# 86885974647565434342125458569795756674/torch.distributed.pipeline.sync.Pipe

Measured on AMD Instinct MI355X. Metric: tokens/sec for 12-layer Transformer at PP=N (pipeline-parallel training), higher is better.
Workload: dtype bf16

## Files before the change

### mipipe/csrc/kernels/attention.hip

```cpp
#include <type_traits>

#include "common.h"
#include "kernels.h"

namespace mipipe {

namespace {

typedef __attribute__((ext_vector_type(4))) short s16x4;
typedef __attribute__((ext_vector_type(8))) short s16x8;
typedef __attribute__((address_space(3))) s16x4 lds_s16x4;

constexpr int kRows = 64;
constexpr int kThreads = 256;
constexpr float kLog2e = 1.4426950408889634f;

template <int D>
struct Img {
  static constexpr int kRowBytes = 2 * D;
  static constexpr int kChunks = D / 8;
  static constexpr int kBytes = kRows * kRowBytes;
  __device__ static __forceinline__ int f(int r) {
    if constexpr (kChunks >= 16) return (((r ^ (r >> 2)) & 1) << 1) | ((r & 2) << 1) | (r & 8);
    else if constexpr (kChunks == 8) return ((((r >> 1) ^ (r >> 2)) & 1) << 1) | ((r >> 1) & 4);
    else return (((r & 3) << 2) | ((r >> 2) & 3)) & (kChunks - 1);
  }
  __device__ static __forceinline__ int off(int r, int c16) { return r * kRowBytes + ((c16 ^ f(r)) << 4); }
};

template <int D>
__device__ __forceinline__ void stage_tile(const bf16_t* __restrict__ base, int64_t ld, char* img, int tid) {
  constexpr int kPer = kRows * Img<D>::kChunks / kThreads;
#pragma unroll
  for (int u = 0; u < kPer; ++u) {
    const int id = tid + u * kThreads;
    const int r = id / Img<D>::kChunks, c = id % Img<D>::kChunks;
    const uint4 v = *reinterpret_cast<const uint4*>(base + (int64_t)r * ld + c * 8);
    *reinterpret_cast<uint4*>(img + Img<D>::off(r, c)) = v;
  }
}

struct TileRegs {
  uint4 r0, r1, r2, r3;
};
template <int D>
__device__ __forceinline__ uint4 load_piece(const bf16_t* __restrict__ base, int64_t ld, int tid, int u) {
  const int id = tid + u * kThreads;
  const int r = id / Img<D>::kChunks, c = id % Img<D>::kChunks;
  return *reinterpret_cast<const uint4*>(base + (int64_t)r * ld + c * 8);
}
template <int D>
__device__ __forceinline__ void store_piece(char* img, int tid, int u, const uint4& v) {
  const int id = tid + u * kThreads;
// ... 904 lines not shown
        float dp = pacc[j][r];
        float pdrop = pr;
        if (a.p > 0.f) {
          const uint32_t w = r == 0 ? kw0 : (r == 1 ? kw1 : (r == 2 ? kw2 : kw3));
          const bool keep = w >= a.threshold;
          pdrop = keep ? pr * pscale : 0.f;
          dp = keep ? dp * pscale : 0.f;
        }
        pd[j][r] = pdrop;
        ds[j][r] = pr * (dp - dl);
        if constexpr (SOFTCAP) ds[j][r] *= dcap;
      }
    }
    scratch_write(scr, pd, lane);
    __builtin_amdgcn_s_waitcnt(0xC07F);
    bf16x8 f0 = scratch_frag(scr, 0, lane);
    bf16x8 f1 = scratch_frag(scr, 1, lane);
#pragma unroll
    for (int t2 = 0; t2 < ND; ++t2) {
      dv[t2] = __builtin_amdgcn_mfma_f32_16x16x32_bf16(f0, frag_cols<D>(dimg, 16 * t2, 0, lane), dv[t2], 0, 0, 0);
      dv[t2] = __builtin_amdgcn_mfma_f32_16x16x32_bf16(f1, frag_cols<D>(dimg, 16 * t2, 1, lane), dv[t2], 0, 0, 0);
    }
    __builtin_amdgcn_s_waitcnt(0xC07F);
    scratch_write(scr, ds, lane);
    __builtin_amdgcn_s_waitcnt(0xC07F);
    f0 = scratch_frag(scr, 0, lane);
    f1 = scratch_frag(scr, 1, lane);
#pragma unroll
    for (int t2 = 0; t2 < ND; ++t2) {
      dk[t2] = __builtin_amdgcn_mfma_f32_16x16x32_bf16(f0, frag_cols<D>(qimg, 16 * t2, 0, lane), dk[t2], 0, 0, 0);
      dk[t2] = __builtin_amdgcn_mfma_f32_16x16x32_bf16(f1, frag_cols<D>(qimg, 16 * t2, 1, lane), dk[t2], 0, 0, 0);
    }
  }
  const DkvDst dst = dkv_dst<0>(blockIdx.y);
  bf16_t* dK = dst.dk;
  bf16_t* dV = dst.dv;
#pragma unroll
  for (int t2 = 0; t2 < ND; ++t2)
#pragma unroll
    for (int r = 0; r < 4; ++r) {
      const int64_t o = (int64_t)(key0 + r) * dst.ld + 16 * t2 + (lane & 15);
      dK[o] = f2bf(dk[t2][r] * a.scale);
      dV[o] = f2bf(dv[t2][r]);
    }
}

namespace shortseq {

constexpr int S = 128;
constexpr int kThreads = 512;
constexpr int kChunk = 64;
constexpr int kChunkImg = S * kChunk * 2;
constexpr int kSqImg = S * S * 2;
constexpr int kStageBytes = 3 * kChunkImg;
constexpr int kPOff = 4 * kChunkImg;
constexpr int kDsOff = kPOff + kSqImg;
constexpr int kSmem = kDsOff + kSqImg;
constexpr int kFwdPOff = 2 * kChunkImg;
constexpr int kFwdSmem = kFwdPOff + kSqImg;

__device__ __forceinline__ int coff(int r, int c16) { return Img<64>::off(r, c16); }
__device__ __forceinline__ int soff(int r, int c16) { return Img<128>::off(r, c16); }

__device__ __forceinline__ void load_chunk(const bf16_t* __restrict__ base, int64_t ld, int d0, int tid, uint4& v0,
                                           uint4& v1) {
  const int r = tid >> 3, c = tid & 7;
  v0 = *reinterpret_cast<const uint4*>(base + (int64_t)r * ld + d0 + 8 * c);
  v1 = *reinterpret_cast<const uint4*>(base + (int64_t)(r + 64) * ld + d0 + 8 * c);
}
__device__ __forceinline__ void store_chunk(char* img, int tid, const uint4& v0, const uint4& v1) {
  const int r = tid >> 3, c = tid & 7;
  *reinterpret_cast<uint4*>(img + coff(r, c)) = v0;
  *reinterpret_cast<uint4*>(img + coff(r + 64, c)) = v1;
}

__device__ __forceinline__ bf16x8 crow(const char* img, int rb, int s, int lane) {
  return *reinterpret_cast<const bf16x8*>(img + coff(rb + (lane & 15), 4 * s + (lane >> 4)));
}
__device__ __forceinline__ bf16x8 ccol(const char* img, int db, int s, int lane) {
  const int g = lane >> 4, q = (lane & 15) >> 2, p = lane & 3;
  const int r0 = 32 * s + 8 * g + q;
  const int c8 = (db >> 2) + p;
  const int o0 = coff(r0, c8 >> 1) + 8 * (c8 & 1);
  const int o1 = coff(r0 + 4, c8 >> 1) + 8 * (c8 & 1);
  const s16x4 lo = __builtin_amdgcn_ds_read_tr16_b64_v4i16((lds_s16x4*)(img + o0));
  const s16x4 hi = __builtin_amdgcn_ds_read_tr16_b64_v4i16((lds_s16x4*)(img + o1));
  return __builtin_bit_cast(bf16x8, __builtin_shufflevector(lo, hi, 0, 1, 2, 3, 4, 5, 6, 7));
}
__device__ __forceinline__ bf16x8 srow(const char* img, int rb, int s, int lane) {
  return *reinterpret_cast<const bf16x8*>(img + soff(rb + (lane & 15), 4 * s + (lane >> 4)));
}
__device__ __forceinline__ bf16x8 scol(const char* img, int ib, int s, int lane) {
  const int g = lane >> 4, q = (lane & 15) >> 2, p = lane & 3;
  const int r0 = 32 * s + 8 * g + q;
  const int c8 = (ib >> 2) + p;
  const int o0 = soff(r0, c8 >> 1) + 8 * (c8 & 1);
  const int o1 = soff(r0 + 4, c8 >> 1) + 8 * (c8 & 1);
  const s16x4 lo = __builtin_amdgcn_ds_read_tr16_b64_v4i16((lds_s16x4*)(img + o0));
  const s16x4 hi = __builtin_amdgcn_ds_read_tr16_b64_v4i16((lds_s16x4*)(img + o1));
  return __builtin_bit_cast(bf16x8, __builtin_shufflevector(lo, hi, 0, 1, 2, 3, 4, 5, 6, 7));
}

template <int D, bool CAUSAL>
__global__ void __launch_bounds__(kThreads, 1) attn_bwd_s128_kernel(AttnArgs a) {
  extern __shared__ __attribute__((aligned(16))) char smem[];
  const int tid = threadIdx.x, lane = tid & 63, wave = __builtin_amdgcn_readfirstlane(tid >> 6);
  const int bh = blockIdx.x;
  const int b = bh / a.H, h = bh % a.H;
  const int64_t boff = (int64_t)b * a.sb_qkv + (int64_t)h * a.sh_qkv;
  const int64_t koff = (int64_t)b * a.sb_qkv + (int64_t)kv_head(a, h) * a.sh_qkv;
  const bf16_t* Q = reinterpret_cast<const bf16_t*>(a.q) + boff;
  const bf16_t* K = reinterpret_cast<const bf16_t*>(a.k) + koff;
  const bf16_t* V = reinterpret_cast<const bf16_t*>(a.v) + koff;
  const bf16_t* dO = reinterpret_cast<const bf16_t*>(a.dout) + (int64_t)b * a.sb_o + (int64_t)h * a.sh_o;
  constexpr int NC = D / kChunk;

  f32x4 sacc[8], pacc[8];
#pragma unroll
  for (int j = 0; j < 8; ++j) sacc[j] = pacc[j] = f32x4{0.f, 0.f, 0.f, 0.f};
  const int myrow = wave * 16 + (lane & 15);
  const bf16_t* qrow = Q + (int64_t)myrow * a.ld_qkv;
  const bf16_t* drow = dO + (int64_t)myrow * a.ld_o;

  uint4 k0, k1, v0, v1;
  load_chunk(K, a.ld_qkv, 0, tid, k0, k1);
  load_chunk(V, a.ld_qkv, 0, tid, v0, v1);
  store_chunk(smem, tid, k0, k1);
  store_chunk(smem + kChunkImg, tid, v0, v1);
  __syncthreads();
#pragma unroll 1
  for (int c = 0; c < NC; ++c) {
    const char* kimg = smem + (c & 1) * 2 * kChunkImg;
    const char* vimg = kimg + kChunkImg;
    if (c + 1 < NC) {
      load_chunk(K, a.ld_qkv, (c + 1) * kChunk, tid, k0, k1);
      load_chunk(V, a.ld_qkv, (c + 1) * kChunk, tid, v0, v1);
    }
    bf16x8 qf[2], df[2];
#pragma unroll
    for (int s2 = 0; s2 < 2; ++s2) {
      qf[s2] = frag_global(qrow + c * kChunk, s2, lane);
      df[s2] = frag_global(drow + c * kChunk, s2, lane);
    }
#pragma unroll
    for (int s2 = 0; s2 < 2; ++s2)
#pragma unroll
      for (int j = 0; j < 8; ++j) {
        sacc[j] = __builtin_amdgcn_mfma_f32_16x16x32_bf16(qf[s2], crow(kimg, 16 * j, s2, lane), sacc[j], 0, 0, 0);
        pacc[j] = __builtin_amdgcn_mfma_f32_16x16x32_bf16(df[s2], crow(vimg, 16 * j, s2, lane), pacc[j], 0, 0, 0);
      }
    if (c + 1 < NC) {
      char* nimg = smem + ((c + 1) & 1) * 2 * kChunkImg;
      store_chunk(nimg, tid, k0, k1);
      store_chunk(nimg + kChunkImg, tid, v0, v1);
    }
    __syncthreads();
  }

  const int qrow0 = wave * 16 + 4 * (lane >> 4);
  const float sl2 = a.scale * kLog2e;
  const float pscale = a.p > 0.f ? 1.f / (1.f - a.p) : 1.f;
  float lse2[4];
#pragma unroll
  for (int r = 0; r < 4; ++r) lse2[r] = a.lse[(int64_t)bh * S + qrow0 + r] * kLog2e;
  float dsum[4] = {0.f, 0.f, 0.f, 0.f};
#pragma unroll
  for (int j = 0; j < 8; ++j) {
    const int key = 16 * j + (lane & 15);
    uint32_t w[4] = {0xFFFFFFFFu, 0xFFFFFFFFu, 0xFFFFFFFFu, 0xFFFFFFFFu};
    if (a.p > 0.f) {
      const uint4 mw = attn_mask_words(a, bh, qrow0 >> 2, key);
      w[0] = mw.x; w[1] = mw.y; w[2] = mw.z; w[3] = mw.w;
    }
#pragma unroll
    for (int r = 0; r < 4; ++r) {
      float pr = __builtin_amdgcn_exp2f(sacc[j][r] * sl2 - lse2[r]);
      if (CAUSAL && key > qrow0 + r) pr = 0.f;
      float dp = pacc[j][r];
      float pd = pr;
      if (a.p > 0.f) {
        const bool keep = w[r] >= a.threshold;
        dp = keep ? dp * pscale : 0.f;
        pd = keep ? pr * pscale : 0.f;
      }
      sacc[j][r] = pr;
      pacc[j][r] = dp;
      dsum[r] += pr * dp;
      *reinterpret_cast<bf16_t*>(smem + kPOff + soff(qrow0 + r, key >> 3) + 2 * (key & 7)) = f2bf(pd);
    }
  }
  float delta[4];
#pragma unroll
  for (int r = 0; r < 4; ++r) delta[r] = row_reduce_sum16(dsum[r]);
#pragma unroll
  for (int j = 0; j < 8; ++j) {
    const int key = 16 * j + (lane & 15);
#pragma unroll
    for (int r = 0; r < 4; ++r) {
      const float ds = sacc[j][r] * (pacc[j][r] - delta[r]);
      *reinterpret_cast<bf16_t*>(smem + kDsOff + soff(qrow0 + r, key >> 3) + 2 * (key & 7)) = f2bf(ds);
    }
  }

  const char* pimg = smem + kPOff;
  const char* dsimg = smem + kDsOff;
  char* kimg = smem;
  char* qimg = smem + kChunkImg;
  char* dimg = smem + 2 * kChunkImg;
  const int r0 = wave * 16;
  uint4 a0, a1, b0, b1, e0, e1;
  load_chunk(K, a.ld_qkv, 0, tid, a0, a1);
  load_chunk(Q, a.ld_qkv, 0, tid, b0, b1);
  load_chunk(dO, a.ld_o, 0, tid, e0, e1);
#pragma unroll 1
  for (int c = 0; c < NC; ++c) {
    const int d0 = c * kChunk;
    __syncthreads();
    store_chunk(kimg, tid, a0, a1);
    store_chunk(qimg, tid, b0, b1);
    store_chunk(dimg, tid, e0, e1);
    __syncthreads();
    if (c + 1 < NC) {
      load_chunk(K, a.ld_qkv, d0 + kChunk, tid, a0, a1);
      load_chunk(Q, a.ld_qkv, d0 + kChunk, tid, b0, b1);
      load_chunk(dO, a.ld_o, d0 + kChunk, tid, e0, e1);
    }
    f32x4 dq[4], dk[4], dv[4];
#pragma unroll
    for (int t = 0; t < 4; ++t) dq[t] = dk[t] = dv[t] = f32x4{0.f, 0.f, 0.f, 0.f};
#pragma unroll
    for (int ks = 0; ks < 4; ++ks) {
      const bf16x8 a_dq = srow(dsimg, r0, ks, lane);
      const bf16x8 a_dk = scol(dsimg, r0, ks, lane);
      const bf16x8 a_dv = scol(pimg, r0, ks, lane);
#pragma unroll
      for (int t = 0; t < 4; ++t) {
        dq[t] = __builtin_amdgcn_mfma_f32_16x16x32_bf16(a_dq, ccol(kimg, 16 * t, ks, lane), dq[t], 0, 0, 0);
        dk[t] = __builtin_amdgcn_mfma_f32_16x16x32_bf16(a_dk, ccol(qimg, 16 * t, ks, lane), dk[t], 0, 0, 0);
        dv[t] = __builtin_amdgcn_mfma_f32_16x16x32_bf16(a_dv, ccol(dimg, 16 * t, ks, lane), dv[t], 0, 0, 0);
      }
    }
    const int orow = r0 + 4 * (lane >> 4);
    __syncthreads();
#pragma unroll
    for (int t = 0; t < 4; ++t) {
      const int col = 16 * t + (lane & 15);
#pragma unroll
      for (int r = 0; r < 4; ++r) {
        const int at = coff(orow + r, col >> 3) + 2 * (col & 7);
        *reinterpret_cast<bf16_t*>(kimg + at) = f2bf(dq[t][r] * a.scale);
        *reinterpret_cast<bf16_t*>(qimg + at) = f2bf(dk[t][r] * a.scale);
        *reinterpret_cast<bf16_t*>(dimg + at) = f2bf(dv[t][r]);
      }
    }
    __syncthreads();
    {
      const int r = tid >> 3, cc = tid & 7;
      const DkvDst dst = dkv_dst<0>(blockIdx.x);
      bf16_t* dK = dst.dk;
      bf16_t* dV = dst.dv;
      bf16_t* dQ = dq_dst<0>(blockIdx.x);
#pragma unroll
      for (int h2 = 0; h2 < 2; ++h2) {
        const int row = r + 64 * h2;
        const int off = coff(row, cc);
        const int64_t g = (int64_t)row * a.ld_qkv + d0 + 8 * cc;
        const int64_t gk = (int64_t)row * dst.ld + d0 + 8 * cc;
        *reinterpret_cast<uint4*>(dQ + g) = *reinterpret_cast<const uint4*>(kimg + off);
        *reinterpret_cast<uint4*>(dK + gk) = *reinterpret_cast<const uint4*>(qimg + off);
        *reinterpret_cast<uint4*>(dV + gk) = *reinterpret_cast<const uint4*>(dimg + off);
      }
    }
  }
}

template <int D, bool CAUSAL>
__global__ void __launch_bounds__(kThreads, 2) attn_fwd_s128_kernel(AttnArgs a) {
  extern __shared__ __attribute__((aligned(16))) char smem[];
  const int tid = threadIdx.x, lane = tid & 63, wave = __builtin_amdgcn_readfirstlane(tid >> 6);
  const int bh = blockIdx.x;
  const int b = bh / a.H, h = bh % a.H;
  const int64_t boff = (int64_t)b * a.sb_qkv + (int64_t)h * a.sh_qkv;
  const int64_t koff = (int64_t)b * a.sb_qkv + (int64_t)kv_head(a, h) * a.sh_qkv;
  const bf16_t* Q = reinterpret_cast<const bf16_t*>(a.q) + boff;
  const bf16_t* K = reinterpret_cast<const bf16_t*>(a.k) + koff;
  const bf16_t* V = reinterpret_cast<const bf16_t*>(a.v) + koff;
  constexpr int NC = D / kChunk;

  f32x4 sacc[8];
#pragma unroll
  for (int j = 0; j < 8; ++j) sacc[j] = f32x4{0.f, 0.f, 0.f, 0.f};
  const bf16_t* qrow = Q + (int64_t)(wave * 16 + (lane & 15)) * a.ld_qkv;

  uint4 k0, k1;
  load_chunk(K, a.ld_qkv, 0, tid, k0, k1);
  store_chunk(smem, tid, k0, k1);
  __syncthreads();
#pragma unroll 1
  for (int c = 0; c < NC; ++c) {
    const char* kimg = smem + (c & 1) * kChunkImg;
    if (c + 1 < NC) load_chunk(K, a.ld_qkv, (c + 1) * kChunk, tid, k0, k1);
    bf16x8 qf[2];
#pragma unroll
    for (int s2 = 0; s2 < 2; ++s2) qf[s2] = frag_global(qrow + c * kChunk, s2, lane);
#pragma unroll
    for (int s2 = 0; s2 < 2; ++s2)
#pragma unroll
      for (int j = 0; j < 8; ++j)
        sacc[j] = __builtin_amdgcn_mfma_f32_16x16x32_bf16(qf[s2], crow(kimg, 16 * j, s2, lane), sacc[j], 0, 0, 0);
    if (c + 1 < NC) store_chunk(smem + ((c + 1) & 1) * kChunkImg, tid, k0, k1);
    __syncthreads();
  }

  const int qrow0 = wave * 16 + 4 * (lane >> 4);
  const float sl2 = a.scale * kLog2e;
  const float pscale = a.p > 0.f ? 1.f / (1.f - a.p) : 1.f;
  float mx[4] = {-INFINITY, -INFINITY, -INFINITY, -INFINITY};
#pragma unroll
  for (int j = 0; j < 8; ++j) {
    const int key = 16 * j + (lane & 15);
#pragma unroll
    for (int r = 0; r < 4; ++r) {
      float x = sacc[j][r] * sl2;
      if (CAUSAL && key > qrow0 + r) x = -INFINITY;
      sacc[j][r] = x;
      mx[r] = fmaxf(mx[r], x);
    }
  }
#pragma unroll
  for (int r = 0; r < 4; ++r) mx[r] = row_reduce_max16(mx[r]);
  float sum[4] = {0.f, 0.f, 0.f, 0.f};
#pragma unroll
  for (int j = 0; j < 8; ++j)
#pragma unroll
    for (int r = 0; r < 4; ++r) {
      const float e = __builtin_amdgcn_exp2f(sacc[j][r] - mx[r]);
      sacc[j][r] = e;
      sum[r] += e;
    }
  float inv[4];
#pragma unroll
  for (int r = 0; r < 4; ++r) {
    sum[r] = row_reduce_sum16(sum[r]);
    inv[r] = 1.f / sum[r];
  }
  char* pimg = smem + kFwdPOff;
#pragma unroll
  for (int j = 0; j < 8; ++j) {
    const int key = 16 * j + (lane & 15);
    uint32_t w[4] = {0xFFFFFFFFu, 0xFFFFFFFFu, 0xFFFFFFFFu, 0xFFFFFFFFu};
    if (a.p > 0.f) {
      const uint4 mw = attn_mask_words(a, bh, qrow0 >> 2, key);
      w[0] = mw.x; w[1] = mw.y; w[2] = mw.z; w[3] = mw.w;
    }
#pragma unroll
    for (int r = 0; r < 4; ++r) {
      float pv = sacc[j][r] * inv[r];
      if (a.p > 0.f) pv = w[r] >= a.threshold ? pv * pscale : 0.f;
      *reinterpret_cast<bf16_t*>(pimg + soff(qrow0 + r, key >> 3) + 2 * (key & 7)) = f2bf(pv);
    }
  }
  if ((lane & 15) == 0) {
#pragma unroll
    for (int r = 0; r < 4; ++r) a.lse[(int64_t)bh * S + qrow0 + r] = (mx[r] + log2f(sum[r])) / kLog2e;
  }

  bf16_t* O = reinterpret_cast<bf16_t*>(a.o) + (int64_t)b * a.sb_o + (int64_t)h * a.sh_o;
  uint4 v0, v1;
  load_chunk(V, a.ld_qkv, 0, tid, v0, v1);
  store_chunk(smem, tid, v0, v1);
  __syncthreads();
  const int r0 = wave * 16;
#pragma unroll 1
  for (int c = 0; c < NC; ++c) {
    const char* vimg = smem + (c & 1) * kChunkImg;
    if (c + 1 < NC) load_chunk(V, a.ld_qkv, (c + 1) * kChunk, tid, v0, v1);
    f32x4 o[4];
#pragma unroll
    for (int t = 0; t < 4; ++t) o[t] = f32x4{0.f, 0.f, 0.f, 0.f};
#pragma unroll
    for (int ks = 0; ks < 4; ++ks) {
      const bf16x8 ap = srow(pimg, r0, ks, lane);
#pragma unroll
      for (int t = 0; t < 4; ++t)
        o[t] = __builtin_amdgcn_mfma_f32_16x16x32_bf16(ap, ccol(vimg, 16 * t, ks, lane), o[t], 0, 0, 0);
    }
    const int orow = r0 + 4 * (lane >> 4);
#pragma unroll
    for (int t = 0; t < 4; ++t)
#pragma unroll
      for (int r = 0; r < 4; ++r)
        O[(int64_t)(orow + r) * a.ld_o + c * kChunk + 16 * t + (lane & 15)] = f2bf(o[t][r]);
    if (c + 1 < NC) store_chunk(smem + ((c + 1) & 1) * kChunkImg, tid, v0, v1);
    __syncthreads();
  }
}

}

template <int D>
size_t fwd_smem() { return 2 * Img<D>::kBytes + 4 * 16 * kScrStride * 2; }
template <int D>
size_t dkdv_smem() { return fwd_smem<D>() + 128 * sizeof(float); }

int g_attn_fused_bwd = 1;
const int g_attn_wide = [] {
  const char* e = getenv("MIPIPE_ATTN_WIDE");
  return e == nullptr ? 1 : atoi(e);
}();

template <typename Kern>
void set_smem(Kern k, size_t bytes) {
  hipFuncSetAttribute(reinterpret_cast<const void*>(k), hipFuncAttributeMaxDynamicSharedMemorySize, (int)bytes);
}

template <int D, bool CAUSAL>
void run_fwd(const AttnArgs& a, hipStream_t s) {
  if (a.S == shortseq::S && g_attn_fused_bwd) {
    static bool once_s = false;
    if (!once_s) {
      set_smem(shortseq::attn_fwd_s128_kernel<D, CAUSAL>, shortseq::kFwdSmem);
      once_s = true;
    }
    hipLaunchKernelGGL((shortseq::attn_fwd_s128_kernel<D, CAUSAL>), dim3(a.B * a.H), dim3(shortseq::kThreads),
                       shortseq::kFwdSmem, s, a);
    return;
  }
  if (D == 64 && a.S % kWideRows == 0 && g_attn_wide) {
    static bool once_w = false;
    if (!once_w) { set_smem(attn_fwd_wide_kernel<CAUSAL>, wide_fwd_smem()); once_w = true; }
    hipLaunchKernelGGL((attn_fwd_wide_kernel<CAUSAL>), dim3(a.S / kWideRows, a.B * a.H), dim3(kThreads),
                       wide_fwd_smem(), s, a);
    return;
  }
  const size_t sm = fwd_smem<D>();
  static bool once = false;
  if (!once) { set_smem(attn_fwd_kernel<D, CAUSAL>, sm); once = true; }
  hipLaunchKernelGGL((attn_fwd_kernel<D, CAUSAL>), dim3(a.S / kRows, a.B * a.H), dim3(kThreads), sm, s, a);
}

template <int D, bool CAUSAL>
void run_bwd(const AttnArgs& a, hipStream_t s) {
  const size_t sm = fwd_smem<D>(), sm2 = dkdv_smem<D>();
  static bool once = false;
  if (!once) {
    set_smem(attn_dq_kernel<D, CAUSAL>, sm);
    set_smem(attn_dkdv_kernel<D, CAUSAL>, sm2);
    once = true;
  }
  if (a.S == shortseq::S && g_attn_fused_bwd) {
    static bool once_s = false;
    if (!once_s) {
      set_smem(shortseq::attn_bwd_s128_kernel<D, CAUSAL>, shortseq::kSmem);
      once_s = true;
    }
    hipLaunchKernelGGL((shortseq::attn_bwd_s128_kernel<D, CAUSAL>), dim3(a.B * a.H), dim3(shortseq::kThreads),
                       shortseq::kSmem, s, a);
    return;
  }
  const int64_t rows = (int64_t)a.B * a.S * a.H;
  hipLaunchKernelGGL(attn_delta_kernel, dim3((unsigned)((rows + 3) / 4)), dim3(256), 0, s, a, D);
  hipLaunchKernelGGL((attn_dkdv_kernel<D, CAUSAL>), dim3(a.S / kRows, a.B * a.H), dim3(kThreads), sm2, s, a);
  if (D == 64 && a.S % kWideRows == 0 && g_attn_wide) {
    static bool once_w = false;
    if (!once_w) { set_smem(attn_dq_wide_kernel<CAUSAL>, wide_fwd_smem()); once_w = true; }
    hipLaunchKernelGGL((attn_dq_wide_kernel<CAUSAL>), dim3(a.S / kWideRows, a.B * a.H), dim3(kThreads),
                       wide_fwd_smem(), s, a);
    return;
  }
  hipLaunchKernelGGL((attn_dq_kernel<D, CAUSAL>), dim3(a.S / kRows, a.B * a.H), dim3(kThreads), sm, s, a);
}

template <int D, bool CAUSAL, bool WINDOW, bool SOFTCAP, bool DOCS, bool SINK>
void launch_fwd_generic(const AttnArgs& a, hipStream_t s) {
  const size_t sm = fwd_smem<D>();
  static bool once = false;
  if (!once) { set_smem(attn_fwd_kernel<D, CAUSAL, WINDOW, SOFTCAP, DOCS, SINK>, sm); once = true; }
  hipLaunchKernelGGL((attn_fwd_kernel<D, CAUSAL, WINDOW, SOFTCAP, DOCS, SINK>), dim3(a.S / kRows, a.B * a.H),
                     dim3(kThreads), sm, s, a);
}

template <int D, bool CAUSAL, bool WINDOW, bool SOFTCAP, bool DOCS>
void launch_bwd_generic(const AttnArgs& a, hipStream_t s) {
  const size_t sm = fwd_smem<D>(), sm2 = dkdv_smem<D>();
  static bool once = false;
  if (!once) {
    set_smem(attn_dq_kernel<D, CAUSAL, WINDOW, SOFTCAP, DOCS>, sm);
    set_smem(attn_dkdv_kernel<D, CAUSAL, WINDOW, SOFTCAP, DOCS>, sm2);
    once = true;
  }
  const dim3 grid(a.S / kRows, a.B * a.H);
  hipLaunchKernelGGL((attn_delta_mfma_kernel<D>), grid, dim3(kThreads), 0, s, a);
  hipLaunchKernelGGL((attn_dkdv_kernel<D, CAUSAL, WINDOW, SOFTCAP, DOCS>), grid, dim3(kThreads), sm2, s, a);
  hipLaunchKernelGGL((attn_dq_kernel<D, CAUSAL, WINDOW, SOFTCAP, DOCS>), grid, dim3(kThreads), sm, s, a);
}

void normalise_window(AttnArgs& a) {
  if (!a.causal || a.window < 0 || a.window >= a.S) a.window = 0;
}

bool normalise_docs(AttnArgs& a) {
  if (a.doc_start == nullptr || a.doc_end == nullptr || !a.causal) {
    a.doc_start = a.doc_end = nullptr;
    return false;
  }
  if (a.window <= 0) a.window = a.S;
  return true;
}

AttnArgs prepared(const AttnArgs& ai) {
// ... 84 lines not shown
```

Baseline: 157,200.

## Keep full K/V resident in LDS and register-cache Q/dO in fused S=128 attention backward

The fused short-sequence backward kernel now loads every K and V head-dim chunk into LDS once, with a two-deep register prefetch, and keeps Q and dO fragments in registers for the whole kernel. The second phase then reuses the resident K image and refills Q/dO from registers instead of reloading K, Q and dO from global memory. The loops are fully unrolled at compile time with precomputed LDS offsets, which cuts global traffic and address arithmetic. In exchange the LDS footprint grows with D, reaching the full 160KB at D=256, and register pressure rises.

```diff
diff --git a/mipipe/csrc/kernels/attention.hip b/mipipe/csrc/kernels/attention.hip
--- a/mipipe/csrc/kernels/attention.hip
+++ b/mipipe/csrc/kernels/attention.hip
@@ -1,4 +1,5 @@
 #include <type_traits>
+#include <utility>
 
 #include "common.h"
 #include "kernels.h"
@@ -1009,53 +1010,61 @@
 constexpr int kChunk = 64;
 constexpr int kChunkImg = S * kChunk * 2;
 constexpr int kSqImg = S * S * 2;
-constexpr int kStageBytes = 3 * kChunkImg;
-constexpr int kPOff = 4 * kChunkImg;
-constexpr int kDsOff = kPOff + kSqImg;
-constexpr int kSmem = kDsOff + kSqImg;
+template <int D>
+struct BwdMap {
+  static constexpr int NC = D / kChunk;
+  static constexpr int kKOff = 0;
+  static constexpr int kVOff = NC * kChunkImg;
+  static constexpr int kPOff = kVOff;
+  static constexpr int kDsOff = kPOff + kSqImg;
+  static constexpr int kQOff = kVOff + (NC * kChunkImg > 2 * kSqImg ? NC * kChunkImg : 2 * kSqImg);
+  static constexpr int kDoOff = kQOff + kChunkImg;
+  static constexpr int kSmem = kDoOff + kChunkImg;
+};
+static_assert(BwdMap<256>::kSmem == 160 * 1024, "D = 256 uses the whole LDS of a CU");
 constexpr int kFwdPOff = 2 * kChunkImg;
 constexpr int kFwdSmem = kFwdPOff + kSqImg;
 
 __device__ __forceinline__ int coff(int r, int c16) { return Img<64>::off(r, c16); }
 __device__ __forceinline__ int soff(int r, int c16) { return Img<128>::off(r, c16); }
 
-__device__ __forceinline__ void load_chunk(const bf16_t* __restrict__ base, int64_t ld, int d0, int tid, uint4& v0,
-                                           uint4& v1) {
+template <typename V>
+__device__ __forceinline__ void load_chunk(const bf16_t* __restrict__ base, int64_t ld, int d0, int tid, V& v0, V& v1) {
   const int r = tid >> 3, c = tid & 7;
-  v0 = *reinterpret_cast<const uint4*>(base + (int64_t)r * ld + d0 + 8 * c);
-  v1 = *reinterpret_cast<const uint4*>(base + (int64_t)(r + 64) * ld + d0 + 8 * c);
-}
-__device__ __forceinline__ void store_chunk(char* img, int tid, const uint4& v0, const uint4& v1) {
+  v0 = *reinterpret_cast<const V*>(base + (int64_t)r * ld + d0 + 8 * c);
+  v1 = *reinterpret_cast<const V*>(base + (int64_t)(r + 64) * ld + d0 + 8 * c);
+}
+template <typename V>
+__device__ __forceinline__ void store_chunk(char* img, int tid, const V& v0, const V& v1) {
   const int r = tid >> 3, c = tid & 7;
-  *reinterpret_cast<uint4*>(img + coff(r, c)) = v0;
-  *reinterpret_cast<uint4*>(img + coff(r + 64, c)) = v1;
+  *reinterpret_cast<V*>(img + coff(r, c)) = v0;
+  *reinterpret_cast<V*>(img + coff(r + 64, c)) = v1;
 }
 
 __device__ __forceinline__ bf16x8 crow(const char* img, int rb, int s, int lane) {
   return *reinterpret_cast<const bf16x8*>(img + coff(rb + (lane & 15), 4 * s + (lane >> 4)));
+}
+__device__ __forceinline__ bf16x8 tr_pair(const char* img, int o0, int o1) {
+  const s16x4 lo = __builtin_amdgcn_ds_read_tr16_b64_v4i16((lds_s16x4*)(img + o0));
+  const s16x4 hi = __builtin_amdgcn_ds_read_tr16_b64_v4i16((lds_s16x4*)(img + o1));
+  return __builtin_bit_cast(bf16x8, __builtin_shufflevector(lo, hi, 0, 1, 2, 3, 4, 5, 6, 7));
 }
 __device__ __forceinline__ bf16x8 ccol(const char* img, int db, int s, int lane) {
   const int g = lane >> 4, q = (lane & 15) >> 2, p = lane & 3;
   const int r0 = 32 * s + 8 * g + q;
   const int c8 = (db >> 2) + p;
-  const int o0 = coff(r0, c8 >> 1) + 8 * (c8 & 1);
-  const int o1 = coff(r0 + 4, c8 >> 1) + 8 * (c8 & 1);
-  const s16x4 lo = __builtin_amdgcn_ds_read_tr16_b64_v4i16((lds_s16x4*)(img + o0));
-  const s16x4 hi = __builtin_amdgcn_ds_read_tr16_b64_v4i16((lds_s16x4*)(img + o1));
-  return __builtin_bit_cast(bf16x8, __builtin_shufflevector(lo, hi, 0, 1, 2, 3, 4, 5, 6, 7));
+  return tr_pair(img, coff(r0, c8 >> 1) + 8 * (c8 & 1), coff(r0 + 4, c8 >> 1) + 8 * (c8 & 1));
 }
 __device__ __forceinline__ bf16x8 srow(const char* img, int rb, int s, int lane) {
   return *reinterpret_cast<const bf16x8*>(img + soff(rb + (lane & 15), 4 * s + (lane >> 4)));
 }
-__device__ __forceinline__ bf16x8 scol(const char* img, int ib, int s, int lane) {
-  const int g = lane >> 4, q = (lane & 15) >> 2, p = lane & 3;
-  const int r0 = 32 * s + 8 * g + q;
-  const int c8 = (ib >> 2) + p;
-  const int o0 = soff(r0, c8 >> 1) + 8 * (c8 & 1);
-  const int o1 = soff(r0 + 4, c8 >> 1) + 8 * (c8 & 1);
-  const s16x4 lo = __builtin_amdgcn_ds_read_tr16_b64_v4i16((lds_s16x4*)(img + o0));
-  const s16x4 hi = __builtin_amdgcn_ds_read_tr16_b64_v4i16((lds_s16x4*)(img + o1));
-  return __builtin_bit_cast(bf16x8, __builtin_shufflevector(lo, hi, 0, 1, 2, 3, 4, 5, 6, 7));
+template <typename F, int... C>
+__device__ __forceinline__ void for_chunks_impl(F&& f, std::integer_sequence<int, C...>) {
+  (f(std::integral_constant<int, C>{}), ...);
+}
+template <int N, typename F>
+__device__ __forceinline__ void for_chunks(F&& f) {
+  for_chunks_impl(f, std::make_integer_sequence<int, N>{});
 }
 
 template <int D, bool CAUSAL>
@@ -1070,56 +1079,83 @@
   const bf16_t* K = reinterpret_cast<const bf16_t*>(a.k) + koff;
   const bf16_t* V = reinterpret_cast<const bf16_t*>(a.v) + koff;
   const bf16_t* dO = reinterpret_cast<const bf16_t*>(a.dout) + (int64_t)b * a.sb_o + (int64_t)h * a.sh_o;
-  constexpr int NC = D / kChunk;
-
-  f32x4 sacc[8], pacc[8];
-#pragma unroll
-  for (int j = 0; j < 8; ++j) sacc[j] = pacc[j] = f32x4{0.f, 0.f, 0.f, 0.f};
+  using M = BwdMap<D>;
+  constexpr int NC = M::NC;
+
   const int myrow = wave * 16 + (lane & 15);
   const bf16_t* qrow = Q + (int64_t)myrow * a.ld_qkv;
   const bf16_t* drow = dO + (int64_t)myrow * a.ld_o;
-
-  uint4 k0, k1, v0, v1;
-  load_chunk(K, a.ld_qkv, 0, tid, k0, k1);
-  load_chunk(V, a.ld_qkv, 0, tid, v0, v1);
-  store_chunk(smem, tid, k0, k1);
-  store_chunk(smem + kChunkImg, tid, v0, v1);
+  const int qrow0 = wave * 16 + 4 * (lane >> 4);
+  constexpr int kDepth = NC < 2 ? NC : 2;
+  bf16x8 kr[kDepth][2], vr[kDepth][2];
+  bf16x8 qf[NC][2], df[NC][2];
+  for_chunks<NC>([&](auto ci) {
+    constexpr int c = decltype(ci)::value;
+    if constexpr (c < kDepth) {
+      load_chunk(K, a.ld_qkv, c * kChunk, tid, kr[c][0], kr[c][1]);
+      load_chunk(V, a.ld_qkv, c * kChunk, tid, vr[c][0], vr[c][1]);
+    }
+#pragma unroll
+    for (int s2 = 0; s2 < 2; ++s2) {
+      qf[c][s2] = frag_global(qrow + c * kChunk, s2, lane);
+      df[c][s2] = frag_global(drow + c * kChunk, s2, lane);
+    }
+  });
+  f32x4 lse2;
+#pragma unroll
+  for (int r = 0; r < 4; ++r) lse2[r] = a.lse[(int64_t)bh * S + qrow0 + r];
+  __builtin_amdgcn_sched_barrier(0);
+
+  f32x4 sacc[8], pacc[8];
+#pragma unroll
+  for (int j = 0; j < 8; ++j) sacc[j] = pacc[j] = f32x4{0.f, 0.f, 0.f, 0.f};
+  int ca[2], cv[2];
+#pragma unroll
+  for (int s2 = 0; s2 < 2; ++s2) {
+    ca[s2] = M::kKOff + coff(lane & 15, 4 * s2 + (lane >> 4));
+    cv[s2] = ca[s2] - M::kKOff + M::kVOff;
+    asm volatile("" : "+v"(cv[s2]));
+  }
+  for_chunks<NC>([&](auto ci) {
+    constexpr int c = decltype(ci)::value;
+    char* kimg = smem + M::kKOff + c * kChunkImg;
+    char* vimg = smem + M::kVOff + c * kChunkImg;
+    constexpr int slot = c % kDepth;
+    store_chunk(kimg, tid, kr[slot][0], kr[slot][1]);
+    store_chunk(vimg, tid, vr[slot][0], vr[slot][1]);
+    if constexpr (c + kDepth < NC) {
+      load_chunk(K, a.ld_qkv, (c + kDepth) * kChunk, tid, kr[slot][0], kr[slot][1]);
+      load_chunk(V, a.ld_qkv, (c + kDepth) * kChunk, tid, vr[slot][0], vr[slot][1]);
+    }
+    __syncthreads();
+#pragma unroll
+    for (int s2 = 0; s2 < 2; ++s2)
+#pragma unroll
+      for (int j = 0; j < 8; ++j) {
+        constexpr int at = c * kChunkImg;
+        const bf16x8 kf = *reinterpret_cast<const bf16x8*>(smem + ca[s2] + at + j * 2048);
+        const bf16x8 vf = *reinterpret_cast<const bf16x8*>(smem + cv[s2] + at + j * 2048);
+        sacc[j] = __builtin_amdgcn_mfma_f32_16x16x32_bf16(qf[c][s2], kf, sacc[j], 0, 0, 0);
+        pacc[j] = __builtin_amdgcn_mfma_f32_16x16x32_bf16(df[c][s2], vf, pacc[j], 0, 0, 0);
+      }
+  });
+  char* qimg = smem + M::kQOff;
+  char* dimg = smem + M::kDoOff;
+  auto fill_qdo = [&](const bf16x8 (&qc)[2], const bf16x8 (&dc)[2]) {
+#pragma unroll
+    for (int s2 = 0; s2 < 2; ++s2) {
+      const int at = coff(myrow, 4 * s2 + (lane >> 4));
+      *reinterpret_cast<bf16x8*>(qimg + at) = qc[s2];
+      *reinterpret_cast<bf16x8*>(dimg + at) = dc[s2];
+    }
+  };
+  fill_qdo(qf[0], df[0]);
   __syncthreads();
-#pragma unroll 1
-  for (int c = 0; c < NC; ++c) {
-    const char* kimg = smem + (c & 1) * 2 * kChunkImg;
-    const char* vimg = kimg + kChunkImg;
-    if (c + 1 < NC) {
-      load_chunk(K, a.ld_qkv, (c + 1) * kChunk, tid, k0, k1);
-      load_chunk(V, a.ld_qkv, (c + 1) * kChunk, tid, v0, v1);
-    }
-    bf16x8 qf[2], df[2];
-#pragma unroll
-    for (int s2 = 0; s2 < 2; ++s2) {
-      qf[s2] = frag_global(qrow + c * kChunk, s2, lane);
-      df[s2] = frag_global(drow + c * kChunk, s2, lane);
-    }
-#pragma unroll
-    for (int s2 = 0; s2 < 2; ++s2)
-#pragma unroll
-      for (int j = 0; j < 8; ++j) {
-        sacc[j] = __builtin_amdgcn_mfma_f32_16x16x32_bf16(qf[s2], crow(kimg, 16 * j, s2, lane), sacc[j], 0, 0, 0);
-        pacc[j] = __builtin_amdgcn_mfma_f32_16x16x32_bf16(df[s2], crow(vimg, 16 * j, s2, lane), pacc[j], 0, 0, 0);
-      }
-    if (c + 1 < NC) {
-      char* nimg = smem + ((c + 1) & 1) * 2 * kChunkImg;
-      store_chunk(nimg, tid, k0, k1);
-      store_chunk(nimg + kChunkImg, tid, v0, v1);
-    }
-    __syncthreads();
-  }
-
-  const int qrow0 = wave * 16 + 4 * (lane >> 4);
+
   const float sl2 = a.scale * kLog2e;
   const float pscale = a.p > 0.f ? 1.f / (1.f - a.p) : 1.f;
-  float lse2[4];
-#pragma unroll
-  for (int r = 0; r < 4; ++r) lse2[r] = a.lse[(int64_t)bh * S + qrow0 + r] * kLog2e;
+#pragma unroll
+  for (int r = 0; r < 4; ++r) lse2[r] *= kLog2e;
   float dsum[4] = {0.f, 0.f, 0.f, 0.f};
 #pragma unroll
   for (int j = 0; j < 8; ++j) {
@@ -1143,7 +1179,7 @@
       sacc[j][r] = pr;
       pacc[j][r] = dp;
       dsum[r] += pr * dp;
-      *reinterpret_cast<bf16_t*>(smem + kPOff + soff(qrow0 + r, key >> 3) + 2 * (key & 7)) = f2bf(pd);
+      *reinterpret_cast<bf16_t*>(smem + M::kPOff + soff(qrow0 + r, key >> 3) + 2 * (key & 7)) = f2bf(pd);
     }
   }
   float delta[4];
@@ -1155,53 +1191,64 @@
 #pragma unroll
     for (int r = 0; r < 4; ++r) {
       const float ds = sacc[j][r] * (pacc[j][r] - delta[r]);
-      *reinterpret_cast<bf16_t*>(smem + kDsOff + soff(qrow0 + r, key >> 3) + 2 * (key & 7)) = f2bf(ds);
-    }
-  }
-
-  const char* pimg = smem + kPOff;
-  const char* dsimg = smem + kDsOff;
-  char* kimg = smem;
-  char* qimg = smem + kChunkImg;
-  char* dimg = smem + 2 * kChunkImg;
+      *reinterpret_cast<bf16_t*>(smem + M::kDsOff + soff(qrow0 + r, key >> 3) + 2 * (key & 7)) = f2bf(ds);
+    }
+  }
+
+  const char* dsimg = smem + M::kDsOff;
   const int r0 = wave * 16;
-  uint4 a0, a1, b0, b1, e0, e1;
-  load_chunk(K, a.ld_qkv, 0, tid, a0, a1);
-  load_chunk(Q, a.ld_qkv, 0, tid, b0, b1);
-  load_chunk(dO, a.ld_o, 0, tid, e0, e1);
-#pragma unroll 1
-  for (int c = 0; c < NC; ++c) {
-    const int d0 = c * kChunk;
+  int lane2 = lane, tid2 = tid;
+  asm volatile("" : "+v"(lane2), "+v"(tid2));
+  lane2 &= 63, tid2 &= kThreads - 1;
+  int cb[4], cq[4], sp0, sp1;
+  {
+    const int rb = 8 * (lane2 >> 4) + ((lane2 & 15) >> 2), pp = lane2 & 3;
+#pragma unroll
+    for (int t = 0; t < 4; ++t) {
+      cb[t] = M::kKOff + coff(rb, (4 * t + pp) >> 1) + 8 * (pp & 1);
+      cq[t] = cb[t] - M::kKOff + M::kQOff;
+      asm volatile("" : "+v"(cq[t]));
+    }
+    const int c8 = (r0 >> 2) + pp;
+    sp0 = M::kPOff + soff(rb, c8 >> 1) + 8 * (c8 & 1);
+    sp1 = M::kPOff + soff(rb + 4, c8 >> 1) + 8 * (c8 & 1);
+    asm volatile("" : "+v"(sp0), "+v"(sp1));
+  }
+  constexpr int kDo = M::kDoOff - M::kQOff, kDs = M::kDsOff - M::kPOff;
+  for_chunks<NC>([&](auto ci) {
+    constexpr int c = decltype(ci)::value;
+    constexpr int d0 = c * kChunk;
+    char* kimg = smem + M::kKOff + c * kChunkImg;
+    if constexpr (c > 0) {
+      __syncthreads();
+      fill_qdo(qf[c], df[c]);
+    }
     __syncthreads();
-    store_chunk(kimg, tid, a0, a1);
-    store_chunk(qimg, tid, b0, b1);
-    store_chunk(dimg, tid, e0, e1);
+    f32x4 dq[4], dk[4], dv[4];
+#pragma unroll
+    for (int t = 0; t < 4; ++t) dq[t] = dk[t] = dv[t] = f32x4{0.f, 0.f, 0.f, 0.f};
+#pragma unroll
+    for (int ks = 0; ks < 4; ++ks) {
+      const bf16x8 a_dq = srow(dsimg, r0, ks, lane2);
+      const bf16x8 a_dk = tr_pair(smem, sp0 + kDs + ks * 8192, sp1 + kDs + ks * 8192);
+      const bf16x8 a_dv = tr_pair(smem, sp0 + ks * 8192, sp1 + ks * 8192);
+#pragma unroll
+      for (int t = 0; t < 4; ++t) {
+        constexpr int k0 = c * kChunkImg;
+        const int o0 = ks * 4096, o1 = 512 + ks * 4096;
+        dq[t] = __builtin_amdgcn_mfma_f32_16x16x32_bf16(a_dq, tr_pair(smem, cb[t] + k0 + o0, cb[t ^ 1] + k0 + o1),
+                                                        dq[t], 0, 0, 0);
+        dk[t] = __builtin_amdgcn_mfma_f32_16x16x32_bf16(a_dk, tr_pair(smem, cq[t] + o0, cq[t ^ 1] + o1), dk[t], 0, 0, 0);
+        dv[t] = __builtin_amdgcn_mfma_f32_16x16x32_bf16(a_dv, tr_pair(smem, cq[t] + kDo + o0, cq[t ^ 1] + kDo + o1),
+                                                        dv[t], 0, 0, 0);
+      }
+      if constexpr (NC == 4) __builtin_amdgcn_sched_barrier(0);
+    }
+    const int orow = r0 + 4 * (lane2 >> 4);
     __syncthreads();
-    if (c + 1 < NC) {
-      load_chunk(K, a.ld_qkv, d0 + kChunk, tid, a0, a1);
-      load_chunk(Q, a.ld_qkv, d0 + kChunk, tid, b0, b1);
-      load_chunk(dO, a.ld_o, d0 + kChunk, tid, e0, e1);
-    }
-    f32x4 dq[4], dk[4], dv[4];
-#pragma unroll
-    for (int t = 0; t < 4; ++t) dq[t] = dk[t] = dv[t] = f32x4{0.f, 0.f, 0.f, 0.f};
-#pragma unroll
-    for (int ks = 0; ks < 4; ++ks) {
-      const bf16x8 a_dq = srow(dsimg, r0, ks, lane);
-      const bf16x8 a_dk = scol(dsimg, r0, ks, lane);
-      const bf16x8 a_dv = scol(pimg, r0, ks, lane);
-#pragma unroll
-      for (int t = 0; t < 4; ++t) {
-        dq[t] = __builtin_amdgcn_mfma_f32_16x16x32_bf16(a_dq, ccol(kimg, 16 * t, ks, lane), dq[t], 0, 0, 0);
-        dk[t] = __builtin_amdgcn_mfma_f32_16x16x32_bf16(a_dk, ccol(qimg, 16 * t, ks, lane), dk[t], 0, 0, 0);
-        dv[t] = __builtin_amdgcn_mfma_f32_16x16x32_bf16(a_dv, ccol(dimg, 16 * t, ks, lane), dv[t], 0, 0, 0);
-      }
-    }
-    const int orow = r0 + 4 * (lane >> 4);
-    __syncthreads();
 #pragma unroll
     for (int t = 0; t < 4; ++t) {
-      const int col = 16 * t + (lane & 15);
+      const int col = 16 * t + (lane2 & 15);
 #pragma unroll
       for (int r = 0; r < 4; ++r) {
         const int at = coff(orow + r, col >> 3) + 2 * (col & 7);
@@ -1212,7 +1259,7 @@
     }
     __syncthreads();
     {
-      const int r = tid >> 3, cc = tid & 7;
+      const int r = tid2 >> 3, cc = tid2 & 7;
       const DkvDst dst = dkv_dst<0>(blockIdx.x);
       bf16_t* dK = dst.dk;
       bf16_t* dV = dst.dv;
@@ -1228,7 +1275,7 @@
         *reinterpret_cast<uint4*>(dV + gk) = *reinterpret_cast<const uint4*>(dimg + off);
       }
     }
-  }
+  });
 }
 
 template <int D, bool CAUSAL>
@@ -1408,11 +1455,11 @@
   if (a.S == shortseq::S && g_attn_fused_bwd) {
     static bool once_s = false;
     if (!once_s) {
-      set_smem(shortseq::attn_bwd_s128_kernel<D, CAUSAL>, shortseq::kSmem);
+      set_smem(shortseq::attn_bwd_s128_kernel<D, CAUSAL>, shortseq::BwdMap<D>::kSmem);
       once_s = true;
     }
     hipLaunchKernelGGL((shortseq::attn_bwd_s128_kernel<D, CAUSAL>), dim3(a.B * a.H), dim3(shortseq::kThreads),
-                       shortseq::kSmem, s, a);
+                       shortseq::BwdMap<D>::kSmem, s, a);
     return;
   }
   const int64_t rows = (int64_t)a.B * a.S * a.H;
```

Result: no change. 157,600, median of 6 (+0.3%).

## Deepen prefetch and fully unroll chunk loops in S=128 attention kernels

Applied to the files above, without the earlier changes.

Fully unrolls the head-dim chunk loops in the S=128 attention forward and backward kernels using compile-time lambdas. Global loads of K/V now run two chunks ahead with double-buffered registers, Q/dO fragments are hoisted, and LDS operand reads are batched ahead of the MFMAs, with sched_barriers pinning the order. The forward output is staged through LDS so each thread writes 16-byte vectors instead of scattered bf16 stores. The aim is to hide global memory latency and cut store transactions, at the cost of higher register pressure and code size.

```diff
diff --git a/mipipe/csrc/kernels/attention.hip b/mipipe/csrc/kernels/attention.hip
--- a/mipipe/csrc/kernels/attention.hip
+++ b/mipipe/csrc/kernels/attention.hip
@@ -1058,6 +1058,23 @@
   return __builtin_bit_cast(bf16x8, __builtin_shufflevector(lo, hi, 0, 1, 2, 3, 4, 5, 6, 7));
 }
 
+template <int I, int N, typename F>
+__device__ __forceinline__ void unrolled_from(F& f) {
+  if constexpr (I < N) {
+    f(std::integral_constant<int, I>{});
+    unrolled_from<I + 1, N>(f);
+  }
+}
+template <int N, typename F>
+__device__ __forceinline__ void unrolled(F f) {
+  unrolled_from<0, N>(f);
+}
+template <int I>
+__device__ __forceinline__ uint4& pick(uint4& x0, uint4& x1) {
+  if constexpr (I == 0) return x0;
+  else return x1;
+}
+
 template <int D, bool CAUSAL>
 __global__ void __launch_bounds__(kThreads, 1) attn_bwd_s128_kernel(AttnArgs a) {
   extern __shared__ __attribute__((aligned(16))) char smem[];
@@ -1079,47 +1096,75 @@
   const bf16_t* qrow = Q + (int64_t)myrow * a.ld_qkv;
   const bf16_t* drow = dO + (int64_t)myrow * a.ld_o;
 
-  uint4 k0, k1, v0, v1;
-  load_chunk(K, a.ld_qkv, 0, tid, k0, k1);
-  load_chunk(V, a.ld_qkv, 0, tid, v0, v1);
-  store_chunk(smem, tid, k0, k1);
-  store_chunk(smem + kChunkImg, tid, v0, v1);
+  const int qrow0 = wave * 16 + 4 * (lane >> 4);
+  uint4 kA0, kA1, kB0, kB1, vA0, vA1, vB0, vB1;
+  bf16x8 qf[NC][2], df[NC][2];
+  float lse_in[4];
+  load_chunk(K, a.ld_qkv, 0, tid, kA0, kA1);
+  load_chunk(V, a.ld_qkv, 0, tid, vA0, vA1);
+  unrolled<NC>([&](auto ic) {
+    constexpr int c = decltype(ic)::value;
+    if constexpr (c == 1) {
+      load_chunk(K, a.ld_qkv, kChunk, tid, kB0, kB1);
+      load_chunk(V, a.ld_qkv, kChunk, tid, vB0, vB1);
+    }
+    qf[c][0] = frag_global(qrow + c * kChunk, 0, lane);
+    df[c][0] = frag_global(drow + c * kChunk, 0, lane);
+    qf[c][1] = frag_global(qrow + c * kChunk, 1, lane);
+    df[c][1] = frag_global(drow + c * kChunk, 1, lane);
+  });
+#pragma unroll
+  for (int r = 0; r < 4; ++r) lse_in[r] = a.lse[(int64_t)bh * S + qrow0 + r];
+  __builtin_amdgcn_sched_barrier(0);
+  uint4 a0, a1, b0, b1, e0, e1;
+  store_chunk(smem, tid, kA0, kA1);
+  store_chunk(smem + kChunkImg, tid, vA0, vA1);
   __syncthreads();
-#pragma unroll 1
-  for (int c = 0; c < NC; ++c) {
+  unrolled<NC>([&](auto ic) {
+    constexpr int c = decltype(ic)::value;
     const char* kimg = smem + (c & 1) * 2 * kChunkImg;
     const char* vimg = kimg + kChunkImg;
-    if (c + 1 < NC) {
-      load_chunk(K, a.ld_qkv, (c + 1) * kChunk, tid, k0, k1);
-      load_chunk(V, a.ld_qkv, (c + 1) * kChunk, tid, v0, v1);
-    }
-    bf16x8 qf[2], df[2];
-#pragma unroll
-    for (int s2 = 0; s2 < 2; ++s2) {
-      qf[s2] = frag_global(qrow + c * kChunk, s2, lane);
-      df[s2] = frag_global(drow + c * kChunk, s2, lane);
-    }
-#pragma unroll
-    for (int s2 = 0; s2 < 2; ++s2)
-#pragma unroll
-      for (int j = 0; j < 8; ++j) {
-        sacc[j] = __builtin_amdgcn_mfma_f32_16x16x32_bf16(qf[s2], crow(kimg, 16 * j, s2, lane), sacc[j], 0, 0, 0);
-        pacc[j] = __builtin_amdgcn_mfma_f32_16x16x32_bf16(df[s2], crow(vimg, 16 * j, s2, lane), pacc[j], 0, 0, 0);
-      }
-    if (c + 1 < NC) {
+    if constexpr (c + 2 < NC) {
+      load_chunk(K, a.ld_qkv, (c + 2) * kChunk, tid, pick<c & 1>(kA0, kB0), pick<c & 1>(kA1, kB1));
+      load_chunk(V, a.ld_qkv, (c + 2) * kChunk, tid, pick<c & 1>(vA0, vB0), pick<c & 1>(vA1, vB1));
+    }
+    if constexpr (c == NC - 1) {
+      load_chunk(K, a.ld_qkv, 0, tid, a0, a1);
+      load_chunk(Q, a.ld_qkv, 0, tid, b0, b1);
+      load_chunk(dO, a.ld_o, 0, tid, e0, e1);
+    }
+    __builtin_amdgcn_sched_barrier(0);
+    unrolled<2>([&](auto is) {
+      constexpr int s2 = decltype(is)::value;
+#pragma unroll
+      for (int j0 = 0; j0 < 8; j0 += 4) {
+        bf16x8 kb[4], vb[4];
+#pragma unroll
+        for (int jj = 0; jj < 4; ++jj) {
+          kb[jj] = crow(kimg, 16 * (j0 + jj), s2, lane);
+          vb[jj] = crow(vimg, 16 * (j0 + jj), s2, lane);
+        }
+#pragma unroll
+        for (int jj = 0; jj < 4; ++jj) {
+          const int j = j0 + jj;
+          sacc[j] = __builtin_amdgcn_mfma_f32_16x16x32_bf16(qf[c][s2], kb[jj], sacc[j], 0, 0, 0);
+          pacc[j] = __builtin_amdgcn_mfma_f32_16x16x32_bf16(df[c][s2], vb[jj], pacc[j], 0, 0, 0);
+        }
+      }
+    });
+    if constexpr (c + 1 < NC) {
       char* nimg = smem + ((c + 1) & 1) * 2 * kChunkImg;
-      store_chunk(nimg, tid, k0, k1);
-      store_chunk(nimg + kChunkImg, tid, v0, v1);
+      store_chunk(nimg, tid, pick<(c + 1) & 1>(kA0, kB0), pick<(c + 1) & 1>(kA1, kB1));
+      store_chunk(nimg + kChunkImg, tid, pick<(c + 1) & 1>(vA0, vB0), pick<(c + 1) & 1>(vA1, vB1));
     }
     __syncthreads();
-  }
-
-  const int qrow0 = wave * 16 + 4 * (lane >> 4);
+  });
+
   const float sl2 = a.scale * kLog2e;
   const float pscale = a.p > 0.f ? 1.f / (1.f - a.p) : 1.f;
   float lse2[4];
 #pragma unroll
-  for (int r = 0; r < 4; ++r) lse2[r] = a.lse[(int64_t)bh * S + qrow0 + r] * kLog2e;
+  for (int r = 0; r < 4; ++r) lse2[r] = lse_in[r] * kLog2e;
   float dsum[4] = {0.f, 0.f, 0.f, 0.f};
 #pragma unroll
   for (int j = 0; j < 8; ++j) {
@@ -1165,11 +1210,7 @@
   char* qimg = smem + kChunkImg;
   char* dimg = smem + 2 * kChunkImg;
   const int r0 = wave * 16;
-  uint4 a0, a1, b0, b1, e0, e1;
-  load_chunk(K, a.ld_qkv, 0, tid, a0, a1);
-  load_chunk(Q, a.ld_qkv, 0, tid, b0, b1);
-  load_chunk(dO, a.ld_o, 0, tid, e0, e1);
-#pragma unroll 1
+#pragma unroll
   for (int c = 0; c < NC; ++c) {
     const int d0 = c * kChunk;
     __syncthreads();
@@ -1182,6 +1223,7 @@
       load_chunk(Q, a.ld_qkv, d0 + kChunk, tid, b0, b1);
       load_chunk(dO, a.ld_o, d0 + kChunk, tid, e0, e1);
     }
+    __builtin_amdgcn_sched_barrier(0);
     f32x4 dq[4], dk[4], dv[4];
 #pragma unroll
     for (int t = 0; t < 4; ++t) dq[t] = dk[t] = dv[t] = f32x4{0.f, 0.f, 0.f, 0.f};
@@ -1190,11 +1232,18 @@
       const bf16x8 a_dq = srow(dsimg, r0, ks, lane);
       const bf16x8 a_dk = scol(dsimg, r0, ks, lane);
       const bf16x8 a_dv = scol(pimg, r0, ks, lane);
+      bf16x8 bk[4], bq[4], bd[4];
 #pragma unroll
       for (int t = 0; t < 4; ++t) {
-        dq[t] = __builtin_amdgcn_mfma_f32_16x16x32_bf16(a_dq, ccol(kimg, 16 * t, ks, lane), dq[t], 0, 0, 0);
-        dk[t] = __builtin_amdgcn_mfma_f32_16x16x32_bf16(a_dk, ccol(qimg, 16 * t, ks, lane), dk[t], 0, 0, 0);
-        dv[t] = __builtin_amdgcn_mfma_f32_16x16x32_bf16(a_dv, ccol(dimg, 16 * t, ks, lane), dv[t], 0, 0, 0);
+        bk[t] = ccol(kimg, 16 * t, ks, lane);
+        bq[t] = ccol(qimg, 16 * t, ks, lane);
+        bd[t] = ccol(dimg, 16 * t, ks, lane);
+      }
+#pragma unroll
+      for (int t = 0; t < 4; ++t) {
+        dq[t] = __builtin_amdgcn_mfma_f32_16x16x32_bf16(a_dq, bk[t], dq[t], 0, 0, 0);
+        dk[t] = __builtin_amdgcn_mfma_f32_16x16x32_bf16(a_dk, bq[t], dk[t], 0, 0, 0);
+        dv[t] = __builtin_amdgcn_mfma_f32_16x16x32_bf16(a_dv, bd[t], dv[t], 0, 0, 0);
       }
     }
     const int orow = r0 + 4 * (lane >> 4);
@@ -1249,25 +1298,50 @@
   for (int j = 0; j < 8; ++j) sacc[j] = f32x4{0.f, 0.f, 0.f, 0.f};
   const bf16_t* qrow = Q + (int64_t)(wave * 16 + (lane & 15)) * a.ld_qkv;
 
-  uint4 k0, k1;
-  load_chunk(K, a.ld_qkv, 0, tid, k0, k1);
-  store_chunk(smem, tid, k0, k1);
+  uint4 kA0, kA1, kB0, kB1, vA0, vA1, vB0, vB1;
+  bf16x8 qf[NC][2];
+  load_chunk(K, a.ld_qkv, 0, tid, kA0, kA1);
+  unrolled<NC>([&](auto ic) {
+    constexpr int c = decltype(ic)::value;
+    if constexpr (c == 1) load_chunk(K, a.ld_qkv, kChunk, tid, kB0, kB1);
+    if constexpr (c < 2) {
+      qf[c][0] = frag_global(qrow + c * kChunk, 0, lane);
+      qf[c][1] = frag_global(qrow + c * kChunk, 1, lane);
+    }
+  });
+  __builtin_amdgcn_sched_barrier(0);
+  store_chunk(smem, tid, kA0, kA1);
   __syncthreads();
-#pragma unroll 1
-  for (int c = 0; c < NC; ++c) {
+  unrolled<NC>([&](auto ic) {
+    constexpr int c = decltype(ic)::value;
     const char* kimg = smem + (c & 1) * kChunkImg;
-    if (c + 1 < NC) load_chunk(K, a.ld_qkv, (c + 1) * kChunk, tid, k0, k1);
-    bf16x8 qf[2];
-#pragma unroll
-    for (int s2 = 0; s2 < 2; ++s2) qf[s2] = frag_global(qrow + c * kChunk, s2, lane);
-#pragma unroll
-    for (int s2 = 0; s2 < 2; ++s2)
-#pragma unroll
-      for (int j = 0; j < 8; ++j)
-        sacc[j] = __builtin_amdgcn_mfma_f32_16x16x32_bf16(qf[s2], crow(kimg, 16 * j, s2, lane), sacc[j], 0, 0, 0);
-    if (c + 1 < NC) store_chunk(smem + ((c + 1) & 1) * kChunkImg, tid, k0, k1);
+    if constexpr (c == NC - 1) {
+      load_chunk(V, a.ld_qkv, 0, tid, vA0, vA1);
+      __builtin_amdgcn_sched_barrier(0);
+    }
+    unrolled<2>([&](auto is) {
+      constexpr int s2 = decltype(is)::value;
+#pragma unroll
+      for (int j0 = 0; j0 < 8; j0 += 4) {
+        bf16x8 kb[4];
+#pragma unroll
+        for (int jj = 0; jj < 4; ++jj) kb[jj] = crow(kimg, 16 * (j0 + jj), s2, lane);
+#pragma unroll
+        for (int jj = 0; jj < 4; ++jj)
+          sacc[j0 + jj] = __builtin_amdgcn_mfma_f32_16x16x32_bf16(qf[c][s2], kb[jj], sacc[j0 + jj], 0, 0, 0);
+      }
+    });
+    if constexpr (c + 1 < NC)
+      store_chunk(smem + ((c + 1) & 1) * kChunkImg, tid, pick<(c + 1) & 1>(kA0, kB0), pick<(c + 1) & 1>(kA1, kB1));
+    if constexpr (c + 2 < NC) {
+      __builtin_amdgcn_sched_barrier(0);
+      load_chunk(K, a.ld_qkv, (c + 2) * kChunk, tid, pick<c & 1>(kA0, kB0), pick<c & 1>(kA1, kB1));
+      qf[c + 2][0] = frag_global(qrow + (c + 2) * kChunk, 0, lane);
+      qf[c + 2][1] = frag_global(qrow + (c + 2) * kChunk, 1, lane);
+      __builtin_amdgcn_sched_barrier(0);
+    }
     __syncthreads();
-  }
+  });
 
   const int qrow0 = wave * 16 + 4 * (lane >> 4);
   const float sl2 = a.scale * kLog2e;
@@ -1323,34 +1397,56 @@
   }
 
   bf16_t* O = reinterpret_cast<bf16_t*>(a.o) + (int64_t)b * a.sb_o + (int64_t)h * a.sh_o;
-  uint4 v0, v1;
-  load_chunk(V, a.ld_qkv, 0, tid, v0, v1);
-  store_chunk(smem, tid, v0, v1);
+  if constexpr (NC > 1) {
+    load_chunk(V, a.ld_qkv, kChunk, tid, vB0, vB1);
+    __builtin_amdgcn_sched_barrier(0);
+  }
+  store_chunk(smem, tid, vA0, vA1);
   __syncthreads();
   const int r0 = wave * 16;
-#pragma unroll 1
-  for (int c = 0; c < NC; ++c) {
+  unrolled<NC>([&](auto ic) {
+    constexpr int c = decltype(ic)::value;
     const char* vimg = smem + (c & 1) * kChunkImg;
-    if (c + 1 < NC) load_chunk(V, a.ld_qkv, (c + 1) * kChunk, tid, v0, v1);
+    char* oimg = smem + ((c + 1) & 1) * kChunkImg;
+    if constexpr (c + 2 < NC) {
+      load_chunk(V, a.ld_qkv, (c + 2) * kChunk, tid, pick<c & 1>(vA0, vB0), pick<c & 1>(vA1, vB1));
+      __builtin_amdgcn_sched_barrier(0);
+    }
     f32x4 o[4];
 #pragma unroll
     for (int t = 0; t < 4; ++t) o[t] = f32x4{0.f, 0.f, 0.f, 0.f};
 #pragma unroll
     for (int ks = 0; ks < 4; ++ks) {
       const bf16x8 ap = srow(pimg, r0, ks, lane);
-#pragma unroll
-      for (int t = 0; t < 4; ++t)
-        o[t] = __builtin_amdgcn_mfma_f32_16x16x32_bf16(ap, ccol(vimg, 16 * t, ks, lane), o[t], 0, 0, 0);
+      bf16x8 bv[4];
+#pragma unroll
+      for (int t = 0; t < 4; ++t) bv[t] = ccol(vimg, 16 * t, ks, lane);
+#pragma unroll
+      for (int t = 0; t < 4; ++t) o[t] = __builtin_amdgcn_mfma_f32_16x16x32_bf16(ap, bv[t], o[t], 0, 0, 0);
     }
     const int orow = r0 + 4 * (lane >> 4);
 #pragma unroll
-    for (int t = 0; t < 4; ++t)
+    for (int t = 0; t < 4; ++t) {
+      const int col = 16 * t + (lane & 15);
 #pragma unroll
       for (int r = 0; r < 4; ++r)
-        O[(int64_t)(orow + r) * a.ld_o + c * kChunk + 16 * t + (lane & 15)] = f2bf(o[t][r]);
-    if (c + 1 < NC) store_chunk(smem + ((c + 1) & 1) * kChunkImg, tid, v0, v1);
+        *reinterpret_cast<bf16_t*>(oimg + coff(orow + r, col >> 3) + 2 * (col & 7)) = f2bf(o[t][r]);
+    }
     __syncthreads();
-  }
+    {
+      const int r = tid >> 3, cc = tid & 7;
+#pragma unroll
+      for (int h2 = 0; h2 < 2; ++h2) {
+        const int row = r + 64 * h2;
+        *reinterpret_cast<uint4*>(O + (int64_t)row * a.ld_o + c * kChunk + 8 * cc) =
+            *reinterpret_cast<const uint4*>(oimg + coff(row, cc));
+      }
+    }
+    if constexpr (c + 1 < NC) {
+      store_chunk(oimg, tid, pick<(c + 1) & 1>(vA0, vB0), pick<(c + 1) & 1>(vA1, vB1));
+      __syncthreads();
+    }
+  });
 }
 
 }
```

Measured after the change: 158,400 before, 158,900 after, median of 6. Within noise of the previous version (+0.3%).
